# steve-the-bayesian/BOOM

Hardware: AMD Instinct MI355X
Metric: Gibbs sweeps/sec (all chains), n=1e4 p=512 spike-slab (higher is better)
Workload: dtype f64; 1 GPU; BregVsSampler spike-and-slab n=1e4 p=512, 1024 chains per GPU, fp64 (BASELINE configs[1]); chains_per_gpu=1024, true_signals=16, burn_in=1000, parallelism=chains sharded, 1 GPU(s), suf_build=single device MFMA syrk

## Files before the change

boom_amd/csrc/engine.hip:

```cpp
#include "engine_internal.h"

namespace boom_amd {

static thread_local std::string g_error = "";

int fail(int code, const std::string &msg) {
  g_error = msg;
  return code;
}

}

namespace {


const char *status_message(int st) {
  switch (st) {
    case CHAIN_NOT_PD:
      return "The posterior information matrix is not positive definite.  "
             "Check your data or consider adjusting your prior.";
    case CHAIN_NEGATIVE_SS:
      return "Illegal data caused negative sum of squares in "
             "Breg::set_reg_post_params.";
    case CHAIN_ILLEGAL_START:
// ... 1496 lines not shown
  return BA_OK;
}
int read_per_chain(ba_engine *e, const double *dev, int64_t chain, double *out) {
  HIP_TRY(hipStreamSynchronize(e->stream));
  if (chain < 0) HIP_TRY(hipMemcpy(out, dev, (size_t)e->cfg.chains * 8, hipMemcpyDeviceToHost));
  else HIP_TRY(hipMemcpy(out, dev + chain, 8, hipMemcpyDeviceToHost));
  return BA_OK;
}

static int sweep_impl(ba_engine *e, int32_t nsweeps, bool record, int la_half) {
  if (nsweeps < 0) return fail(BA_E_INVALID, "nsweeps must be non-negative");
  int rc = sweep_refusal(e, DATA_REGRESSION);
  if (rc) return rc;
  rc = switch_mode(e, 0, 1.0);
  if (rc) return rc;
  rc = upload_shared(e);
  if (rc) return rc;
  rc = alloc_chain_state(e);
  if (rc) return rc;
  if (record && e->trace_stride > 0 && nsweeps > e->trace_stride)
    return fail(BA_E_INVALID, "nsweeps exceeds the enabled trace length");
  HIP_TRY(e->dmodel.resize(2 * (size_t)e->cfg.chains * ssvs_scalar_layout(64).total));
  SsvsParams P;
  fill_params(e, P);
  if (!record) {
    P.trace_sigsq = P.trace_logp = P.trace_k = nullptr;
    P.rec_idx = nullptr;
    P.rec_beta = nullptr;
    P.trace_stride = 0;
    P.trace_idx = nullptr;
    if (e->trace_stride > 0)
      HIP_TRY(hipMemsetAsync(e->dtrace_idx.ptr, 0, (size_t)e->cfg.chains * 4, e->stream));
  }
  const SsvsLds lay = ssvs_lds_layout(e->p, e->kcap);
  if (lay.total > e->lds_per_cu)
    return fail(BA_E_INVALID, "problem does not fit the LDS working set");
  if (record && e->trace_stride > 0 && la_half < 0)
    HIP_TRY(hipMemsetAsync(e->dtrace_idx.ptr, 0, (size_t)e->cfg.chains * 4, e->stream));
  if (la_half >= 0) {
    const size_t C = (size_t)e->cfg.chains, pp = (size_t)e->p;
    const size_t o1 = (size_t)la_half * C, op = (size_t)la_half * C * pp;
    P.trace_row0 = la_half * e->la_len;
    P.snap_gamma = e->snap_gamma.ptr + op;
    P.snap_beta = e->snap_beta.ptr + op;
    P.snap_sigsq = e->snap_sigsq.ptr + o1;
    P.snap_perm = e->snap_perm.ptr + op;
    P.snap_pos = e->snap_pos.ptr + o1;
    P.snap_fail = e->snap_fail.ptr + o1;
    P.snap_inc = e->snap_inc.ptr + op;
    P.snap_bsum = e->snap_bsum.ptr + op;
    P.snap_bsumsq = e->snap_bsumsq.ptr + op;
    P.snap_acc = e->snap_acc.ptr + (size_t)la_half * C * ACC_COUNT;
  }
#ifndef BA_PIPELINE
#define BA_PIPELINE 1
#endif
  const int resident_per_cu = (int)std::min<size_t>(4, e->lds_per_cu / lay.total);
  const bool pipelined = BA_PIPELINE && nsweeps > 0 && (e->trace_stride == 0 || la_half >= 0) && !e->big_active &&
                         e->cfg.chains <= resident_per_cu * e->cu_count && (!e->kt_enabled || e->kt_overlap);
  if (la_half >= 0 && !pipelined) return fail(BA_E_STATE, "look-ahead batch cannot overlap");
  if (!pipelined) {
    const int C = e->cfg.chains, group = resident_per_cu * e->cu_count;
    const bool groups = BA_PIPELINE && nsweeps > 0 && e->cur_mode != 2 && !e->big_active && C > group &&
                        e->trace_stride == 0 && (!e->kt_enabled || e->kt_overlap);
    if (groups) {
      if (!e->pipe_stream) {
        {
// ... 61 lines not shown
  e->model_ok = true;
  return BA_OK;
}
}

extern "C" {

int ba_sweep(ba_engine *e, int32_t nsweeps) {
  ENGINE_PROLOGUE_NOJOIN(e);
  if (e->la_served < e->la_avail || e->data_kind != DATA_REGRESSION || e->cur_mode != 0) {
    int rcj = pipe_join(e);
    if (rcj) return rcj;
  }
  int rc = la_rewind(e);
  if (rc) return rc;
  return sweep_impl(e, nsweeps, e->la_len <= 1);
}

int ba_set_lookahead(ba_engine *e, int32_t lookahead) {
  ENGINE_PROLOGUE(e);
  if (lookahead < 1) return fail(BA_E_INVALID, "lookahead must be at least 1");
  MUTATE(e);
  if (lookahead > 1) {
    int rc = ba_enable_draws(e, 2 * lookahead);
    if (rc) return rc;
  }
  e->la_len = lookahead;
  e->la_pipe = true;
  return BA_OK;
}

static bool la_can_overlap(const ba_engine *e) {
  if (!BA_PIPELINE || !e->la_pipe || e->big_active || (e->kt_enabled && !e->kt_overlap) || e->kcap <= 0) return false;
  const size_t lds = ssvs_lds_layout(e->p, e->kcap).total;
  if (lds > e->lds_per_cu) return false;
  const int resident_per_cu = (int)std::min<size_t>(4, e->lds_per_cu / lds);
  return e->cfg.chains <= resident_per_cu * e->cu_count;
}

int ba_draw_next(ba_engine *e) {
  ENGINE_PROLOGUE_NOJOIN(e);
  if (e->la_len <= 1) return ba_sweep(e, 1);
  if (e->la_served == e->la_avail) {
    if (e->la_ahead) {
      e->la_slot ^= 1;
      e->la_ahead = false;
      e->la_avail = e->la_served = 0;
      e->la_cache.clear();
      e->la_synced = false;
      e->la_cur_piped = true;
    } else {
      int rc = pipe_join(e);
      if (rc) return rc;
      la_discard(e);
      rc = switch_mode(e, 0, 1.0);
      if (!rc) rc = upload_shared(e);
      if (!rc) rc = alloc_chain_state(e);
      if (rc) return rc;
      if (!e->la_done[0]) {
        HIP_TRY(hipEventCreateWithFlags(&e->la_done[0], hipEventDisableTiming));
        HIP_TRY(hipEventCreateWithFlags(&e->la_done[1], hipEventDisableTiming));
      }
      e->la_slot = 0;
      if (la_can_overlap(e)) {
        rc = la_snap_alloc(e);
        if (!rc) rc = sweep_impl(e, e->la_len, true, 0);
        e->la_cur_piped = true;
// ... 455 lines not shown
```

boom_amd/csrc/ssvs_device.h:

```cpp
#pragma once
#include <hip/hip_runtime.h>

#include "device_rng.h"
#include "diag.h"
#include "ssvs_params.h"

namespace boom_amd {

namespace {

constexpr int WAVE = 64;
#define BA_INF (__builtin_inf())


#define AS_LDS __attribute__((address_space(3)))
typedef AS_LDS double lds_f64;
typedef AS_LDS uint16_t lds_u16;
typedef AS_LDS uint32_t lds_u32;
typedef AS_LDS uint8_t lds_u8;
template <class T>
__device__ __forceinline__ AS_LDS T *to_lds(unsigned char *generic) {
  return (AS_LDS T *)(uintptr_t)generic;
}
#define AS_CONST __attribute__((address_space(4)))
// ... 894 lines not shown
  if (candidate < 0) {
    *status = CHAIN_RNG_BRANCH;
    return;
  }
  double rev;
  {
    const int l2 = P.cm_start[candidate], h2 = P.cm_start[candidate + 1];
    double ans = -BA_INF, tot = 0.0;
    for (int i = l2; i < h2; ++i) {
      const int v = P.cm_idx[i];
      const bool inc = (v == candidate) ? true : ((v == index) ? false : (bool)ch.gam[v]);
      if (!inc) {
        if (v == index) ans = P.cm_cor[i];
        tot += P.cm_cor[i];
      }
    }
    rev = (tot == 0.0) ? 0.0 : ans / tot;
  }
  pe.kind = EV_TRY_LT;
  pe.f1 = index;
  pe.f2 = candidate;
  pe.lfw = log(forward_w);
  pe.lrev = log(rev);
  pe.lu = log(d_runif(rng, 0.0, 1.0));
  pe.check_legal = false;
}

}


enum : int { CMD_EXIT = 0, CMD_EVAL = 1, CMD_UNIF = 2, CMD_DECIDE = 3, CMD_SHUFFLE_DECIDE = 4 };
enum : int { CT_CMD = 0, CT_K = 1, CT_I0 = 2, CT_LOGP = 3, CT_LP = 4, CT_LDV = 5,
             CT_LDA = 6, CT_Q = 7, CT_C = 8, CT_NFLIPS = 9, CT_POS = 10, CT_PERMSEL = 12,
             CT_EVMODE = 13, CT_CUR = 14,
             CT_SLOT0 = 16, CT_SLOT_STRIDE = 6, CT_ROLL = 44, CT_ACC = 48 };
enum : int { SL_F = 0, SL_J = 1, SL_KIND = 2, SL_LOGU = 3, SL_MARGIN = 4, SL_DELTA = 5 };
enum : int { STOP_ACCEPT = 1, STOP_SLOW = 2, STOP_BAD = 3 };

__device__ __forceinline__ void shuffle_targets(const PhiloxKey &key, uint64_t pos,
                                                int p, int tid, int nthreads,
                                                lds_u16 *oth, bool whole_range = false) {
  const int nt = whole_range ? p : p - 1;
  const uint64_t b0 = pos >> 1, b1 = (pos + (uint64_t)(nt - 1)) >> 1;
  for (uint64_t b = b0 + (uint64_t)tid; b <= b1; b += (uint64_t)nthreads) {
    double u[2];
    philox_pair(key, b, &u[0], &u[1]);
#pragma unroll
    for (int h = 0; h < 2; ++h) {
      const long long t = (long long)(2 * b + h) - (long long)pos;
      if (t >= 0 && t < nt) {
        if (whole_range) {
          oth[t] = (uint16_t)(int)floor(0.0 + ((double)p - 0.0) * u[h]);
        } else {
          const int i = p - 1 - (int)t;
          oth[i] = (uint16_t)(int)floor(0.0 + ((double)(i + 1) - 0.0) * u[h]);
        }
      }
    }
  }
}

enum : int { EVM_BATCH = 0, EVM_FILL = 1 };

template <int NB, bool MLVS = false>
__device__ __forceinline__ void eval_share(const SsvsParams &P, Chain &ch,
                                           const Model &M, const PhiloxKey &key,
                                           uint64_t flip_pos, int nflips, int i0,
                                           int evmode, int wave, lds_f64 *ctl,
                                           StampCtx &sx) {
  const int lane = ch.lane;
  SUBSTAMP(sx, 7);
  const int idx = i0 + WAVE * wave + lane;
  if (evmode == EVM_FILL) {
    const bool valid = idx < ch.p;
    const Proposal pr = eval_proposal<NB, true, MLVS>(P, ch, M, valid ? idx : 0, valid, sx, idx - lane);
    if (valid) {
// ... 143 lines not shown
```

boom_amd/csrc/ssvs_kernel.hip:

```cpp
#include "ktimer.h"
#include "ssvs_sweep_body.h"

namespace boom_amd {

__global__ __launch_bounds__(64) void ssvs_logp_kernel(SsvsParams P,
                                                       const uint8_t *gammas,
                                                       int ngamma, double *out,
                                                       int *status_out) {
  extern __shared__ __attribute__((aligned(16))) unsigned char smem[];
  const int which = blockIdx.x, lane = threadIdx.x, p = P.p;
  if (which >= ngamma) return;
  const SsvsLds lay = ssvs_lds_layout(p, P.kcap);
  Chain ch;
  ch.lane = lane;
  ch.p = p;
  bind_lds(ch, smem, lay);
  ch.xty = P.xty;
  ch.DF = P.nobs[0] + P.prior_df;
  ch.ss0q = P.prior_ss + P.yty[0];
  ch.mode = 0;
  ch.sv = ch.sa = ch.sx = 1.0;
  const uint8_t *gg = gammas + (size_t)which * p;
  int k = 0;
  for (int base = 0; base < p; base += WAVE) {
// ... 94 lines not shown
  }
  if (P.snap_gamma) {
    const size_t o = (size_t)chain * (size_t)P.p;
    for (int j = threadIdx.x; j < P.p; j += WAVE * W) {
      P.snap_gamma[o + j] = P.gamma[o + j];
      P.snap_beta[o + j] = P.beta[o + j];
      P.snap_perm[o + j] = P.perm[o + j];
      P.snap_inc[o + j] = P.inc_count[o + j];
      P.snap_bsum[o + j] = P.beta_sum[o + j];
      P.snap_bsumsq[o + j] = P.beta_sumsq[o + j];
    }
    if (threadIdx.x < ACC_COUNT)
      P.snap_acc[(size_t)chain * ACC_COUNT + threadIdx.x] = P.acc[(size_t)chain * ACC_COUNT + threadIdx.x];
    if (threadIdx.x == 0) {
      P.snap_sigsq[chain] = P.sigsq[chain];
      P.snap_pos[chain] = P.rng_pos[chain];
      P.snap_fail[chain] = P.failures[chain];
    }
  }
  ssvs_sweep_body<NB, W, WPE, MLVS>(P, nsweeps, chain, smem);
  if (P.q_out) {
    __syncthreads();
    __threadfence();
    if (threadIdx.x == 0) {
      const int t = atomicAdd(P.q_out + Q_PUSH, 1);
      __hip_atomic_store(P.q_out + Q_READY + t, chain, __ATOMIC_RELEASE, __HIP_MEMORY_SCOPE_AGENT);
    }
  }
}

template <int NB, int W, int WPE, bool MLVS = false>
static hipError_t launch_sweep_t(hipStream_t stream, const SsvsParams &P,
                                 int nsweeps) {
  const SsvsLds lay = ssvs_lds_layout(P.p, NB * 8);
  hipError_t e = hipFuncSetAttribute((const void *)ssvs_sweep_kernel<NB, W, WPE, MLVS>,
                                     hipFuncAttributeMaxDynamicSharedMemorySize,
                                     (int)lay.total);
  if (e != hipSuccess) return e;
  KtScope kt(stream, KT_SSVS);
  hipLaunchKernelGGL((ssvs_sweep_kernel<NB, W, WPE, MLVS>), dim3(P.chain_count), dim3(WAVE * W),
                     lay.total, stream, P, nsweeps);
  return hipGetLastError();
}

hipError_t launch_ssvs_sweep(hipStream_t stream, const SsvsParams &P,
                             int nsweeps) {
  const int key = P.kcap * 10 + P.waves;
#ifndef BA_ONLY_322
  if (P.mode == 3) {
    if (!P.flip_order || !P.wss) return hipErrorInvalidValue;
    switch (P.kcap) {
      case 16: return launch_sweep_t<2, 1, 1, true>(stream, P, nsweeps);
      case 32: return launch_sweep_t<4, 1, 1, true>(stream, P, nsweeps);
      case 48: return launch_sweep_t<6, 1, 1, true>(stream, P, nsweeps);
      case 64: return launch_sweep_t<8, 1, 1, true>(stream, P, nsweeps);
      default: return hipErrorInvalidValue;
    }
  }
#endif
  switch (key) {
#ifdef BA_ONLY_322
    case 322: return launch_sweep_t<4, 2, 2>(stream, P, nsweeps);
    default: return hipErrorInvalidValue;
#else
    case 161: return launch_sweep_t<2, 1, 1>(stream, P, nsweeps);
    case 321: return launch_sweep_t<4, 1, 1>(stream, P, nsweeps);
    case 481: return launch_sweep_t<6, 1, 1>(stream, P, nsweeps);
// ... 63 lines not shown
```

boom_amd/csrc/ssvs_params.h:

```cpp
#pragma once
#include <stdint.h>

namespace boom_amd {

enum ChainStatus : int32_t {
  CHAIN_OK = 0,
  CHAIN_NOT_PD = 1,
  CHAIN_NEGATIVE_SS = 2,
  CHAIN_ILLEGAL_START = 3,
  CHAIN_RNG_BRANCH = 4,
  CHAIN_FORECAST_VARIANCE = 5,
  CHAIN_MODEL_TOO_LARGE = 6,
  CHAIN_NEED_COLUMN = 7,
  CHAIN_NEED_COLUMN_BIG = 8
};
enum { MLVS_ILLEGAL_START = 12 };

enum { SUMMARY_SCALARS = 16 };
enum {
  ACC_SWEEPS = 0,
  ACC_SIGSQ = 1,
  ACC_SIGSQ2 = 2,
  ACC_K = 3,
  ACC_ACCEPTS = 4,
// ... 74 lines not shown
  int32_t trace_stride;
  uint16_t *rec_idx;
  double *rec_beta;
  int32_t rec_cap;

  double *ada_birth, *ada_death;
  uint64_t *ada_iter;
  double ada_step, ada_target;
  int32_t ada_max_flips;
  int32_t *q_in, *q_out;
  int32_t *q_error;
  int32_t trace_row0;
  uint8_t *snap_gamma;
  double *snap_beta, *snap_sigsq, *snap_bsum, *snap_bsumsq, *snap_acc;
  uint16_t *snap_perm;
  uint64_t *snap_pos;
  int32_t *snap_fail;
  uint32_t *snap_inc;
  int32_t adaptive;
  double *ada_ws;

  int32_t big_kcap;
  double *big_model;
  int64_t big_model_stride;
  double *big_xs;
  const double *xty_planes;
  int32_t xty_nplanes;
  int64_t xty_plane_stride;
  const uint16_t *flip_order;
  const double *wss;
};

struct SsvsLds {
  uint32_t Lv, La, rdv, rda, w, bg, ctrl, park, g, perm0, perm1, oth, last, pred, gam, gam0, nbr, total;
};

static inline __host__ __device__ SsvsLds ssvs_lds_layout(int p, int kcap) {
  SsvsLds L;
  const uint32_t nb = (uint32_t)kcap / 8;
  const uint32_t fac = nb * (nb + 1) / 2 * 64 * 8;
  const uint32_t pv = (((uint32_t)p * 2) + 15u) & ~15u;
  uint32_t o = 0;
  L.Lv = o;    o += fac;
  L.La = o;    o += fac;
  L.rdv = o;   o += (uint32_t)kcap * 8;
  L.rda = o;   o += (uint32_t)kcap * 8;
  L.w = o;     o += (uint32_t)kcap * 8;
  L.bg = o;    o += (uint32_t)kcap * 8;
  L.ctrl = o;  o += 512;
  L.park = o;  o += 4 * 512;
  L.g = o;     o += (((uint32_t)kcap * 2) + 15u) & ~15u;
  L.perm0 = o; o += pv;
  L.perm1 = o; o += pv;
  L.oth = o;   o += pv;
  L.last = o;  o += 2 * pv;
  L.pred = o;  o += pv;
  L.gam = o;   o += ((uint32_t)p + 15u) & ~15u;
  L.gam0 = o;  o += ((uint32_t)p + 15u) & ~15u;
  L.nbr = o;   o += ((uint32_t)p + 15u) & ~15u;
  L.total = o;
  return L;
}

struct SsvsBigLds {
  uint32_t tile, rdt, w, y, rd, bst, ctrl, g, gst, perm0, perm1, oth, last, pred, gam, gam0, nbr, total;
};
static inline __host__ __device__ SsvsBigLds ssvs_big_lds_layout(int p, int kcap) {
  SsvsBigLds L;
  const uint32_t pv = (((uint32_t)p * 2) + 15u) & ~15u;
  uint32_t o = 0;
  L.tile = o;  o += 36 * 64 * 8;
  L.rdt = o;   o += 64 * 8;
  L.w = o;     o += (uint32_t)kcap * 8;
  L.y = o;     o += (uint32_t)kcap * 8;
  L.rd = o;    o += (uint32_t)kcap * 8;
  L.bst = o;   o += (uint32_t)kcap * 8;
  L.ctrl = o;  o += 512;
  L.g = o;     o += (((uint32_t)kcap * 2) + 15u) & ~15u;
  L.gst = o;   o += (((uint32_t)kcap * 2) + 15u) & ~15u;
  L.perm0 = o; o += pv;
  L.perm1 = o; o += pv;
  L.oth = o;   o += pv;
  L.last = o;  o += 2 * pv;
  L.pred = o;  o += pv;
  L.gam = o;   o += ((uint32_t)p + 15u) & ~15u;
  L.gam0 = o;  o += ((uint32_t)p + 15u) & ~15u;
  L.nbr = o;   o += ((uint32_t)p + 15u) & ~15u;
  L.total = o;
  return L;
}

struct SsvsAdaLds {
// ... 53 lines not shown
```

boom_amd/csrc/ssvs_sweep_body.h:

```cpp
#pragma once
#include "ssvs_device.h"

namespace boom_amd {

template <int NB, int W, int WPE, bool MLVS = false>
__device__ __forceinline__ void ssvs_sweep_body(SsvsParams P, int nsweeps, const int chain,
                                                unsigned char *smem) {
  constexpr bool SHUFFLE_MASKED = NB >= 6 && W > 1;
  P.V += (size_t)chain * (size_t)P.v_chain_stride;
  if (P.col_valid) {
    P.col_valid += (size_t)chain * (size_t)P.col_words;
    P.v_diag += (size_t)chain * (size_t)P.p;
  }
  int tid_ = threadIdx.x;
  BA_OPAQUE_V(tid_);
  int lane = tid_ & (WAVE - 1);
  const int wave = tid_ >> 6;
  const int p = P.p;
#ifdef BA_PSTAMPS
  long long pst[8];
  pst[0] = (long long)__builtin_readcyclecounter();
#endif
  constexpr int FOLD_Z = 16;
  const bool fold = (W == 1) && P.xty_planes != nullptr;
// ... 1 lines not shown
  double pl[2][FOLD_Z];
  if (fold_early) {
    const double *src = P.xty_planes + (size_t)chain * p;
#pragma unroll
    for (int e = 0; e < 2; ++e) {
      const int j = lane + e * WAVE;
#pragma unroll
      for (int z = 0; z < FOLD_Z; ++z)
        pl[e][z] = (j < p && z < P.xty_nplanes) ? src[(size_t)z * P.xty_plane_stride + j] : 0.0;
    }
  }
  if (P.status[chain] != CHAIN_OK) {
    if (threadIdx.x == 0) {
      P.todo[chain] += nsweeps;
      if (P.ran) P.ran[chain] = 0;
    }
    return;
  }
  int owed_after = 0;
  {
    int total = nsweeps + P.todo[chain];
    if (P.run_limit > 0 && total > P.run_limit) {
      owed_after = total - P.run_limit;
      total = P.run_limit;
    }
    if (total == 0) {
      if (threadIdx.x == 0 && P.ran) P.ran[chain] = 0;
      return;
    }
    nsweeps = total;
  }

  constexpr int KCAP = NB * 8;
  const SsvsLds lay = ssvs_lds_layout(p, KCAP);
  Chain ch;
  ch.lane = lane;
  ch.p = p;
  ch.k = 0;
  bind_lds(ch, smem, lay);
  lds_f64 *ctl = to_lds<double>(smem + lay.ctrl);
  PSTAMP(1);
  ch.xty = P.xty + (size_t)chain * P.xty_stride;
  if (fold_early) {
    double *dst = const_cast<double *>(P.xty) + (size_t)chain * P.xty_stride;
#pragma unroll
    for (int e = 0; e < 2; ++e) {
      const int j = lane + e * WAVE;
      double a = pl[e][0];
#pragma unroll
      for (int z = 1; z < FOLD_Z; ++z)
        if (z < P.xty_nplanes) a += pl[e][z];
      if (j < p) dst[j] = a;
    }
    __builtin_amdgcn_fence(__ATOMIC_RELEASE, "wavefront");
    __builtin_amdgcn_s_waitcnt(0);
  } else if (fold) {
    double *dst = const_cast<double *>(P.xty) + (size_t)chain * P.xty_stride;
    const double *src = P.xty_planes + (size_t)chain * p;
    for (int j = lane; j < p; j += WAVE) {
      double a = src[j];
      for (int z0 = 1; z0 < P.xty_nplanes; z0 += 8) {
        double v[8];
#pragma unroll
        for (int u = 0; u < 8; ++u)
          v[u] = (z0 + u < P.xty_nplanes) ? src[(size_t)(z0 + u) * P.xty_plane_stride + j] : 0.0;
#pragma unroll
        for (int u = 0; u < 8; ++u)
// ... 20 lines not shown
    if (P.slab_scales) { ch.sv = inv; ch.sa = inv; }
  }
  const PhiloxKey key{P.seed_lo, P.seed_hi,
                      (uint32_t)(P.chain_offset + chain), P.stream};

  StampCtx sx_unused;
  sx_unused.last = 0;
  if (W > 1 && wave != 0) {
    sx_unused.last = (long long)__builtin_readcyclecounter();
    for (int i = 0; i < 8; ++i) sx_unused.ph[i] = 0.0;
    for (;;) {
      HSTAMP(sx_unused, 7);
      __syncthreads();
      HSTAMP(sx_unused, 5);
      const int cmd = (int)ctl[CT_CMD];
      if (cmd == CMD_EXIT) break;
      const uint64_t upos = ((AS_LDS const uint64_t *)(ctl + CT_POS))[0];
      if (cmd == CMD_EVAL) {
        Model M;
        M.logp = ctl[CT_LOGP]; M.lp = ctl[CT_LP]; M.ldv = ctl[CT_LDV];
        M.lda = ctl[CT_LDA]; M.Q = ctl[CT_Q]; M.c = ctl[CT_C];
        M.SS = 0; M.pd = true; M.bad = 0;
        ch.k = (int)ctl[CT_K];
        ch.perm = to_lds<uint16_t>(smem + (((int)ctl[CT_PERMSEL]) ? lay.perm1 : lay.perm0));
        bind_slot(ch, P, chain, (int)ctl[CT_CUR]);
        unsigned long long a = (unsigned long long)ch.sc_store;
        asm volatile("" : "+s"(a) : : "memory");
        ch.sc = (c_f64 *)a;
        eval_share<NB, MLVS>(P, ch, M, key, upos, (int)ctl[CT_NFLIPS], (int)ctl[CT_I0],
                             (int)ctl[CT_EVMODE], wave, ctl, sx_unused);
        HSTAMP(sx_unused, 6);
      } else if (cmd == CMD_DECIDE || cmd == CMD_SHUFFLE_DECIDE) {
        if (cmd == CMD_SHUFFLE_DECIDE) {
          shuffle_targets(key, upos, p, threadIdx.x, WAVE * W, ch.oth);
          __syncthreads();
        }
        if (wave == 1) {
          const int sel = (int)ctl[CT_PERMSEL];
          bind_slot(ch, P, chain, (int)ctl[CT_CUR]);
          ch.perm = to_lds<uint16_t>(smem + (sel ? lay.perm1 : lay.perm0));
          ch.perm_alt = to_lds<uint16_t>(smem + (sel ? lay.perm0 : lay.perm1));
          uint64_t fpos = upos;
          if (cmd == CMD_SHUFFLE_DECIDE) {
            parallel_shuffle<SHUFFLE_MASKED>(ch, sx_unused);
            fpos = upos + (uint64_t)(p - 1);
          }
          DecideResult dr;
          decide_walk<MLVS>(ch, key, fpos, (int)ctl[CT_I0], (int)ctl[CT_NFLIPS], dr);
          HSTAMP(sx_unused, 4);
          if (lane == 0) {
            lds_f64 *sl = ctl + CT_SLOT0 + CT_SLOT_STRIDE * 1;
            sl[SL_F] = (double)dr.spos;
            sl[SL_J] = (double)dr.j;
            sl[SL_KIND] = (double)dr.kind;
            sl[SL_LOGU] = dr.logu;
            sl[SL_MARGIN] = dr.margin;
          }
        }
      } else {
        if (p > 1) shuffle_targets(key, upos, p, threadIdx.x, WAVE * W, ch.oth, P.mode == 2);
      }
      HSTAMP(sx_unused, 7);
      __syncthreads();
      HSTAMP(sx_unused, 5);
    }
#if defined(BA_STAMPS) && defined(BA_STAMPS4)
    if (wave == 1 && lane == 0) {
      double *a = P.acc + (size_t)chain * ACC_COUNT;
      for (int i = 0; i < 8; ++i) a[ACC_PHASE0 + i] += sx_unused.ph[i];
    }
#endif
    return;
  }

  uint8_t *g_gamma = P.gamma + (size_t)chain * p;
  uint16_t *g_perm = P.perm + (size_t)chain * p;
  int k = 0;
  int status = CHAIN_OK;
  for (int base = 0; base < p; base += WAVE) {
    const int j = base + lane;
    const int inc = (j < p) ? g_gamma[j] : 0;
    if (j < p) {
      ch.gam[j] = (uint8_t)inc;
      ch.perm[j] = g_perm[j];
      ch.nbr[j] = (uint8_t)((P.cm_start != nullptr) && (P.cm_start[j + 1] > P.cm_start[j]));
    }
    const unsigned long long mask = __ballot(inc != 0);
    const int slot = k + __popcll(mask & ((1ull << lane) - 1ull));
    if (inc && slot < KCAP) ch.g[slot] = (uint16_t)j;
    k += __popcll(mask);
  }
  if (k > KCAP) status = CHAIN_MODEL_TOO_LARGE;
  ch.k = k;
  wave_sync();
  bool aborted = false;
  int need_col = -1;
  int kmax = k;
  int trace_at = (P.trace_row0 >= 0) ? P.trace_row0 : (P.trace_idx ? P.trace_idx[chain] : 0);

  uint64_t pos = uni((uint64_t)P.rng_pos[chain]);
  int failures = uni((int)P.failures[chain]);
  double sigsq = uni((double)P.sigsq[chain]);
  double beta_m = 0.0;
  int gprev = 0, kprev = 0;
  bool beta_valid = false;

  lds_f64 *sum_b = to_lds<double>(smem + lay.park + 512);
  lds_f64 *sum_b2 = to_lds<double>(smem + lay.park + 1024);
  AS_LDS int *sum_n = to_lds<int>(smem + lay.park + 1536);
  AS_LDS int *sum_g = to_lds<int>(smem + lay.park + 1792);
  sum_b[lane] = 0.0; sum_b2[lane] = 0.0; sum_n[lane] = 0; sum_g[lane] = -1;
  if (lane < 8) ctl[CT_ACC + lane] = (lane == ACC_MIN_MARGIN) ? BA_INF : 0.0;
  wave_sync();
#define ACC_ADD(slot, x) do { if (lane == 0) ctl[CT_ACC + (slot)] += (double)(x); } while (0)
#define ACC_MIN(x) do { if (lane == 0) ctl[CT_ACC + ACC_MIN_MARGIN] = fmin(ctl[CT_ACC + ACC_MIN_MARGIN], (x)); } while (0)
  int done = 0;

  const int nflips = P.max_flips;
  STAMP_DECL;
  StampCtx sx;
  sx.last = (long long)__builtin_readcyclecounter();
  for (int i = 0; i < 8; ++i) sx.ph[i] = 0.0;

  Model M;
  M.bad = 0; M.pd = true; M.logp = 0; M.lp = 0; M.ldv = 0; M.lda = 0; M.Q = 0; M.c = 0; M.SS = 0;
  Pending pe;
  pe.kind = EV_INIT; pe.f1 = pe.f2 = -1; pe.lu = 0; pe.lfw = pe.lrev = 0; pe.check_legal = false;
  enum { PH_BEGIN, PH_FLIPS, PH_SWAP, PH_TAIL, PH_JOIN, PH_COMMIT };
  int phase = PH_BEGIN, sweep = 0, i0 = 0;
  bool model_checked = false;
  int perm_sel = 0;
  bool use_table = false;
  int cur = 0, other_var = -1;
  bool other_ok = false, table_valid_other = false;
  const int model_tag_in = P.model_keep ? P.model_tag[chain] : 0;
  const bool model_kept = (model_tag_in & 0xff) == KCAP && status == CHAIN_OK;
  if (model_kept) cur = (model_tag_in >> 8) & 1;
  bind_slot(ch, P, chain, cur);
  bool table_valid = P.table_keep && model_kept && P.table_tag[chain] == model_tag_in;
  int fill_j = 0;
  bool spec = false;
  bool have_dr = false;
  int after_join = PH_COMMIT, spec_status = CHAIN_OK;
  bool commit_pending = false, gam0_fresh = false;
  lds_f64 *park = to_lds<double>(smem + lay.park);
  int stops_prev = table_valid ? 0 : (1 << 20), stops_now = 0;
  uint64_t flip_pos = 0, pos0 = pos;
  WinRng rng;
  rng.init(key, lane, pos);

  PSTAMP(3);
  if (model_kept) {
    {
      const SsvsScalarLayout S = ssvs_scalar_layout(KCAP);
      const double *sc = ch.sc_store + S.scal;
      const double s0 = sc[0], s1 = sc[1], s2 = sc[2], s3 = sc[3], s4 = sc[4], s5 = sc[5], s6 = sc[6], s7 = sc[7];
      restore_model<NB>(ch);
      M.logp = s0; M.lp = s1; M.ldv = s2; M.lda = s3;
      M.Q = s4; M.c = s5; M.SS = s6; M.pd = s7 != 0.0;
      unsigned long long u = (unsigned long long)ch.sc_store;
      asm volatile("s_dcache_inv\n\ts_waitcnt lgkmcnt(0)" : "+s"(u) : : "memory");
      ch.sc = (c_f64 *)u;
    }
    if (P.suf_changed) {
      refactor<true, MLVS>(P, ch, M, sx);
      if (M.bad) status = M.bad;
      else publish_model<NB>(ch, M);
    }
    if (lane == 0) {
      ctl[CT_LOGP] = M.logp; ctl[CT_LP] = M.lp; ctl[CT_LDV] = M.ldv;
      ctl[CT_LDA] = M.lda; ctl[CT_Q] = M.Q; ctl[CT_C] = M.c;
    }
    wave_sync();
    pe.kind = EV_NONE;
  }

  PSTAMP(4);
// ... 109 lines not shown
      if (sweep + (commit_pending ? 1 : 0) >= nsweeps) {
        if (!commit_pending) break;
        phase = PH_COMMIT;
        continue;
      }
      {
        const bool ut = (P.walk_policy != 0) && (stops_prev <= 1 || P.walk_policy == 2);
        const bool mc = model_checked || (M.logp > -BA_INF && M.logp < BA_INF);
        const bool will_fork = nflips > 0 && W > 1 && ut && table_valid && mc && p > 1 && P.walk_policy != 3 && P.mode != 2 && !MLVS;
        if (commit_pending && !will_fork) {
          phase = PH_COMMIT;
          continue;
        }
      }
      STAMP(7);
      TSTAMP(sx, 7);
      if (nflips > 0) {
        if (!gam0_fresh || P.mode) {
          for (int j = lane; j < p; j += WAVE) {
            ch.gam0[j] = ch.gam[j];
            if constexpr (MLVS) ch.perm[j] = P.flip_order[j];
            else if (P.mode) ch.perm[j] = (uint16_t)j;
          }
          gam0_fresh = true;
        }
        TSTAMP(sx, 1);
        pos0 = pos;
        if (!model_checked && M.logp > -BA_INF && M.logp < BA_INF) model_checked = true;
        use_table = (P.walk_policy != 0) && (stops_prev <= 1 || P.walk_policy == 2);
        stops_prev = stops_now;
        stops_now = 0;
        if (W > 1 && use_table && table_valid && model_checked && p > 1 && P.walk_policy != 3 && P.mode != 2 && !MLVS) {
          wave_sync();
          if (lane == 0) {
            ctl[CT_CMD] = (double)CMD_SHUFFLE_DECIDE;
            ctl[CT_I0] = 0.0;
            ctl[CT_NFLIPS] = (double)nflips;
            ctl[CT_PERMSEL] = (double)perm_sel;
            ctl[CT_CUR] = (double)cur;
            ((AS_LDS uint64_t *)(ctl + CT_POS))[0] = pos;
          }
          __syncthreads();
          shuffle_targets(key, pos, p, threadIdx.x, WAVE * W, ch.oth);
          __syncthreads();
          {
            lds_u16 *tmp = ch.perm;
            ch.perm = ch.perm_alt;
            ch.perm_alt = tmp;
            perm_sel ^= 1;
          }
          flip_pos = pos + (uint64_t)(p - 1);
          pos = flip_pos + (uint64_t)nflips;
          TSTAMP(sx, 2);
          spec = true;
          spec_status = CHAIN_OK;
          park[lane] = beta_m;
          if (lane == 0) {
            ctl[CT_ROLL + 0] = sigsq;
            ctl[CT_ROLL + 1] = (double)failures;
            ctl[CT_ROLL + 2] = beta_valid ? 1.0 : 0.0;
          }
          i0 = 0;
          phase = commit_pending ? PH_COMMIT : PH_SWAP;
          STAMP(1);
          continue;
        }
        if constexpr (MLVS) {
          wave_sync();
          flip_pos = pos;
          pos = flip_pos + (uint64_t)nflips;
          if (!(M.logp > -BA_INF && M.logp < BA_INF)) { status = MLVS_ILLEGAL_START; aborted = true; }
        } else {
        if (W > 1) {
          if (lane == 0) {
            ctl[CT_CMD] = (double)CMD_UNIF;
            ((AS_LDS uint64_t *)(ctl + CT_POS))[0] = pos;
          }
// ... 27 lines not shown
                if (!inc && column_missing(P, j)) { status = CHAIN_NEED_COLUMN; need_col = j; aborted = true; break; }
                apply_flip(ch, j);
              }
            }
            pe.kind = EV_INIT;
            pe.check_legal = true;
          }
        }
        }
      }
      i0 = 0;
      phase = PH_FLIPS;
      continue;
    }

    if (phase == PH_FLIPS) {
      if (nflips == 0 || i0 >= nflips) {
        phase = PH_SWAP;
        continue;
      }
      if (use_table && table_valid) {
        DecideResult dr;
        if (W > 1) {
          if (!have_dr) {
          if (lane == 0) {
            ctl[CT_CMD] = (double)CMD_DECIDE;
            ctl[CT_I0] = (double)i0;
            ctl[CT_NFLIPS] = (double)nflips;
            ctl[CT_PERMSEL] = (double)perm_sel;
            ctl[CT_CUR] = (double)cur;
            ((AS_LDS uint64_t *)(ctl + CT_POS))[0] = flip_pos;
          }
          __syncthreads();
          __syncthreads();
          }
          have_dr = false;
          const lds_f64 *sl = ctl + CT_SLOT0 + CT_SLOT_STRIDE * 1;
          dr.spos = uni((int)sl[SL_F]);
          dr.j = uni((int)sl[SL_J]);
          dr.kind = uni((int)sl[SL_KIND]);
          dr.logu = uni((double)sl[SL_LOGU]);
          dr.margin = uni((double)sl[SL_MARGIN]);
        } else {
          decide_walk<MLVS>(ch, key, flip_pos, i0, nflips, dr);
        }
        ACC_MIN(dr.margin);
        STAMP(3);
        if (dr.spos < 0) {
          ACC_ADD(ACC_PROPOSALS, nflips - i0);
          i0 = nflips;
          continue;
        }
        ACC_ADD(ACC_PROPOSALS, dr.spos + 1 - i0);
        ++stops_now;
        i0 = dr.spos + 1;
        if (dr.kind == STOP_BAD) {
          status = CHAIN_NEGATIVE_SS;
          break;
        }
        if (!ch.gam[dr.j] && ch.k >= KCAP) {
          status = CHAIN_MODEL_TOO_LARGE;
          aborted = true;
          break;
        }
        if (!ch.gam[dr.j] && column_missing(P, dr.j)) {
          status = CHAIN_NEED_COLUMN;
// ... 86 lines not shown
      if (kind == STOP_ACCEPT) {
        pe.kind = EV_FORCE;
      } else {
        pe.kind = EV_TRY_GE;
        pe.lu = uni((double)sl[SL_LOGU]);
      }
      i0 += nprop;
      continue;
    }

    if (phase == PH_SWAP) {
      TSTAMP(sx, 7);
      rng.set_pos(pos);
      if (nflips > 0) propose_swap(P, ch, rng, pe, &status);
      pos = rng.get_pos();
      phase = PH_TAIL;
      if (spec && (pe.kind != EV_NONE || status != CHAIN_OK)) {
        spec_status = status;
        status = CHAIN_OK;
        after_join = PH_TAIL;
        phase = PH_JOIN;
      }
      STAMP(4);
      TSTAMP(sx, 3);
      continue;
    }

    if (phase == PH_JOIN) {
      __syncthreads();
      spec = false;
      const lds_f64 *sl = ctl + CT_SLOT0 + CT_SLOT_STRIDE * 1;
      if ((int)sl[SL_F] < 0) {
        ACC_MIN(sl[SL_MARGIN]);
        ACC_ADD(ACC_PROPOSALS, nflips);
        status = spec_status;
        phase = after_join;
        if (after_join == PH_COMMIT && status == CHAIN_OK) {
          commit_pending = true;
          phase = PH_BEGIN;
        }
      } else {
        pos = flip_pos + (uint64_t)nflips;
        beta_m = park[lane];
        sigsq = ctl[CT_ROLL + 0];
        failures = (int)ctl[CT_ROLL + 1];
        beta_valid = ctl[CT_ROLL + 2] != 0.0;
        pe.kind = EV_NONE; pe.f1 = pe.f2 = -1; pe.lfw = pe.lrev = 0.0; pe.check_legal = false;
        have_dr = true;
        phase = PH_FLIPS;
      }
      STAMP(3);
      continue;
    }

    if (phase == PH_COMMIT) {
      TSTAMP(sx, 7);
      k = ch.k;
      gprev = (lane < k) ? (int)ch.g[lane] : 0;
      kprev = k;
      kmax = k > kmax ? k : kmax;
      {
        const int gnow = (lane < k) ? gprev : -1;
        const int gold = sum_g[lane];
        if (__any(gnow != gold)) {
          const int n_old = sum_n[lane];
          if (gold >= 0 && n_old) {
            const size_t o = (size_t)chain * p + gold;
// ... 58 lines not shown
        continue;
      }
      failures = 0;
      const double z = draw_normals(rng, k);
      pos = uni(rng.get_pos());
      TSTAMP(sx, 5);
      const double sigma = P.mode ? 1.0 : sqrt(sigsq);
      double y = (lane < k) ? ch.w[lane] + sigma * z : 0.0;
      const double rdm = (lane < k) ? ch.rdv[lane] : 0.0;
#pragma nounroll
      for (int ib = (k - 1) >> 3; ib >= 0; --ib) {
        double lr[8];
        const int base = bidx(ib * 8, lane < ib * 8 + 8 ? lane : 0);
#pragma unroll
        for (int t = 0; t < 8; ++t) lr[t] = ch.Lv[base + t * 8];
#pragma unroll
        for (int t = 7; t >= 0; --t) {
          const int i = ib * 8 + t;
          if (i < k) {
            const double xi = bcast_u(y * rdm, i);
            if (lane == i) y = xi;
            else if (lane < i) y -= lr[t] * xi;
          }
        }
      }
      beta_m = y;
      beta_valid = true;
      TSTAMP(sx, 6);
    } else if (P.draw_beta) {
      beta_valid = true;
    }
    STAMP(6);
    after_join = PH_COMMIT;
    phase = spec ? PH_JOIN : PH_COMMIT;
  }

  PSTAMP(5);
  if (W > 1) {
    if (lane == 0) ctl[CT_CMD] = (double)CMD_EXIT;
    __syncthreads();
  }

  wave_sync();
#ifndef BA_STAMPS
  double *acc_row = P.acc + (size_t)chain * ACC_COUNT;
  const double acc_old = (lane < 8) ? acc_row[lane] : 0.0;
#endif
  if (sum_g[lane] >= 0 && sum_n[lane]) {
    const size_t o = (size_t)chain * p + sum_g[lane];
    P.inc_count[o] += (unsigned)sum_n[lane];
    P.beta_sum[o] += sum_b[lane];
    P.beta_sumsq[o] += sum_b2[lane];
  }
  wave_sync();
  {
    const lds_u8 *gsrc = aborted ? ch.gam0 : ch.gam;
    const lds_u16 *psrc = (aborted && p > 1) ? ch.perm_alt : ch.perm;
    for (int j = lane; j < p; j += WAVE) {
      g_gamma[j] = gsrc[j];
      g_perm[j] = psrc[j];
    }
    if (aborted) pos = pos0;
  }
  if (beta_valid) {
    double *g_beta = P.beta + (size_t)chain * p;
    for (int j = lane; j < p; j += WAVE) g_beta[j] = 0.0;
// ... 55 lines not shown
```

Baseline: 57.06 million sweeps/s.

## Double-buffer shuffle targets and prefetch next sweep's shuffle during speculation

Adds a second LDS buffer for the shuffle-target array. When the chain is speculating, wave 0 uses its idle time at the end of a sweep to precompute the next sweep's Philox shuffle targets into the spare buffer, so the following CMD_SHUFFLE_DECIDE can skip regenerating them. It also lets a mid-walk CMD_DECIDE re-fork speculation (REFORK) instead of waiting for the helper wave, and corrects the proposal count on join to nflips - i0. The cost is extra LDS use, capped at a quarter of a CU, plus added control-flow complexity and the risk that a stale prefetch is consumed.

```diff
diff --git a/boom_amd/csrc/engine.hip b/boom_amd/csrc/engine.hip
--- a/boom_amd/csrc/engine.hip
+++ b/boom_amd/csrc/engine.hip
@@ -1552,7 +1552,7 @@
     if (e->trace_stride > 0)
       HIP_TRY(hipMemsetAsync(e->dtrace_idx.ptr, 0, (size_t)e->cfg.chains * 4, e->stream));
   }
-  const SsvsLds lay = ssvs_lds_layout(e->p, e->kcap);
+  const SsvsLds lay = ssvs_lds_layout(e->p, e->kcap, e->waves);
   if (lay.total > e->lds_per_cu)
     return fail(BA_E_INVALID, "problem does not fit the LDS working set");
   if (record && e->trace_stride > 0 && la_half < 0)
@@ -1680,7 +1680,7 @@
 
 static bool la_can_overlap(const ba_engine *e) {
   if (!BA_PIPELINE || !e->la_pipe || e->big_active || (e->kt_enabled && !e->kt_overlap) || e->kcap <= 0) return false;
-  const size_t lds = ssvs_lds_layout(e->p, e->kcap).total;
+  const size_t lds = ssvs_lds_layout(e->p, e->kcap, e->waves).total;
   if (lds > e->lds_per_cu) return false;
   const int resident_per_cu = (int)std::min<size_t>(4, e->lds_per_cu / lds);
   return e->cfg.chains <= resident_per_cu * e->cu_count;
diff --git a/boom_amd/csrc/ssvs_device.h b/boom_amd/csrc/ssvs_device.h
--- a/boom_amd/csrc/ssvs_device.h
+++ b/boom_amd/csrc/ssvs_device.h
@@ -950,16 +950,19 @@
 enum : int { CMD_EXIT = 0, CMD_EVAL = 1, CMD_UNIF = 2, CMD_DECIDE = 3, CMD_SHUFFLE_DECIDE = 4 };
 enum : int { CT_CMD = 0, CT_K = 1, CT_I0 = 2, CT_LOGP = 3, CT_LP = 4, CT_LDV = 5,
              CT_LDA = 6, CT_Q = 7, CT_C = 8, CT_NFLIPS = 9, CT_POS = 10, CT_PERMSEL = 12,
-             CT_EVMODE = 13, CT_CUR = 14,
+             CT_EVMODE = 13, CT_CUR = 14, CT_OTH = 15,
              CT_SLOT0 = 16, CT_SLOT_STRIDE = 6, CT_ROLL = 44, CT_ACC = 48 };
 enum : int { SL_F = 0, SL_J = 1, SL_KIND = 2, SL_LOGU = 3, SL_MARGIN = 4, SL_DELTA = 5 };
 enum : int { STOP_ACCEPT = 1, STOP_SLOW = 2, STOP_BAD = 3 };
 
 __device__ __forceinline__ void shuffle_targets(const PhiloxKey &key, uint64_t pos,
                                                 int p, int tid, int nthreads,
-                                                lds_u16 *oth, bool whole_range = false) {
+                                                lds_u16 *oth, bool whole_range = false,
+                                                uint32_t blk_first = 0, uint32_t blk_count = 1u << 30) {
   const int nt = whole_range ? p : p - 1;
-  const uint64_t b0 = pos >> 1, b1 = (pos + (uint64_t)(nt - 1)) >> 1;
+  const uint64_t b0 = (pos >> 1) + (uint64_t)blk_first;
+  uint64_t b1 = (pos + (uint64_t)(nt - 1)) >> 1;
+  if (blk_count < (1u << 30) && b0 + (uint64_t)blk_count <= b1) b1 = b0 + (uint64_t)blk_count - 1;
   for (uint64_t b = b0 + (uint64_t)tid; b <= b1; b += (uint64_t)nthreads) {
     double u[2];
     philox_pair(key, b, &u[0], &u[1]);
diff --git a/boom_amd/csrc/ssvs_kernel.hip b/boom_amd/csrc/ssvs_kernel.hip
--- a/boom_amd/csrc/ssvs_kernel.hip
+++ b/boom_amd/csrc/ssvs_kernel.hip
@@ -150,7 +150,7 @@
 template <int NB, int W, int WPE, bool MLVS = false>
 static hipError_t launch_sweep_t(hipStream_t stream, const SsvsParams &P,
                                  int nsweeps) {
-  const SsvsLds lay = ssvs_lds_layout(P.p, NB * 8);
+  const SsvsLds lay = ssvs_lds_layout(P.p, NB * 8, W);
   hipError_t e = hipFuncSetAttribute((const void *)ssvs_sweep_kernel<NB, W, WPE, MLVS>,
                                      hipFuncAttributeMaxDynamicSharedMemorySize,
                                      (int)lay.total);
diff --git a/boom_amd/csrc/ssvs_params.h b/boom_amd/csrc/ssvs_params.h
--- a/boom_amd/csrc/ssvs_params.h
+++ b/boom_amd/csrc/ssvs_params.h
@@ -130,10 +130,12 @@
 };
 
 struct SsvsLds {
-  uint32_t Lv, La, rdv, rda, w, bg, ctrl, park, g, perm0, perm1, oth, last, pred, gam, gam0, nbr, total;
-};
-
-static inline __host__ __device__ SsvsLds ssvs_lds_layout(int p, int kcap) {
+  uint32_t Lv, La, rdv, rda, w, bg, ctrl, park, g, perm0, perm1, oth, last, pred, gam, gam0, nbr, oth1, total;
+};
+
+enum : uint32_t { SSVS_LDS_QUARTER_CU = 40u * 1024u };
+
+static inline __host__ __device__ SsvsLds ssvs_lds_layout(int p, int kcap, int waves = 1) {
   SsvsLds L;
   const uint32_t nb = (uint32_t)kcap / 8;
   const uint32_t fac = nb * (nb + 1) / 2 * 64 * 8;
@@ -156,6 +158,8 @@
   L.gam = o;   o += ((uint32_t)p + 15u) & ~15u;
   L.gam0 = o;  o += ((uint32_t)p + 15u) & ~15u;
   L.nbr = o;   o += ((uint32_t)p + 15u) & ~15u;
+  L.oth1 = L.oth;
+  if (waves > 1 && o + pv <= SSVS_LDS_QUARTER_CU) { L.oth1 = o; o += pv; }
   L.total = o;
   return L;
 }
diff --git a/boom_amd/csrc/ssvs_sweep_body.h b/boom_amd/csrc/ssvs_sweep_body.h
--- a/boom_amd/csrc/ssvs_sweep_body.h
+++ b/boom_amd/csrc/ssvs_sweep_body.h
@@ -57,7 +57,13 @@
   }
 
   constexpr int KCAP = NB * 8;
-  const SsvsLds lay = ssvs_lds_layout(p, KCAP);
+  const SsvsLds lay = ssvs_lds_layout(p, KCAP, W);
+#ifndef BA_PRE_BLOCKS
+#define BA_PRE_BLOCKS (1u << 30)
+#endif
+  constexpr uint32_t PRE_BLOCKS = BA_PRE_BLOCKS;
+  constexpr bool PRE_ALL = PRE_BLOCKS >= (1u << 30);
+  const bool prefetch = W > 1 && !MLVS && lay.oth1 != lay.oth;
   Chain ch;
   ch.lane = lane;
   ch.p = p;
@@ -144,8 +150,15 @@
         HSTAMP(sx_unused, 6);
       } else if (cmd == CMD_DECIDE || cmd == CMD_SHUFFLE_DECIDE) {
         if (cmd == CMD_SHUFFLE_DECIDE) {
-          shuffle_targets(key, upos, p, threadIdx.x, WAVE * W, ch.oth);
-          __syncthreads();
+          const int ow = (int)ctl[CT_OTH];
+          ch.oth = to_lds<uint16_t>(smem + ((ow & 1) ? lay.oth1 : lay.oth));
+          if (!(ow & 2)) {
+            shuffle_targets(key, upos, p, threadIdx.x, WAVE * W, ch.oth);
+            __syncthreads();
+          } else if (!PRE_ALL) {
+            shuffle_targets(key, upos, p, threadIdx.x, WAVE * W, ch.oth, false, PRE_BLOCKS);
+            __syncthreads();
+          }
         }
         if (wave == 1) {
           const int sel = (int)ctl[CT_PERMSEL];
@@ -170,6 +183,7 @@
           }
         }
       } else {
+        ch.oth = to_lds<uint16_t>(smem + ((((int)ctl[CT_OTH]) & 1) ? lay.oth1 : lay.oth));
         if (p > 1) shuffle_targets(key, upos, p, threadIdx.x, WAVE * W, ch.oth, P.mode == 2);
       }
       HSTAMP(sx_unused, 7);
@@ -223,6 +237,7 @@
   AS_LDS int *sum_g = to_lds<int>(smem + lay.park + 1792);
   sum_b[lane] = 0.0; sum_b2[lane] = 0.0; sum_n[lane] = 0; sum_g[lane] = -1;
   if (lane < 8) ctl[CT_ACC + lane] = (lane == ACC_MIN_MARGIN) ? BA_INF : 0.0;
+  if (lane == 0) ctl[CT_OTH] = 0.0;
   wave_sync();
 #define ACC_ADD(slot, x) do { if (lane == 0) ctl[CT_ACC + (slot)] += (double)(x); } while (0)
 #define ACC_MIN(x) do { if (lane == 0) ctl[CT_ACC + ACC_MIN_MARGIN] = fmin(ctl[CT_ACC + ACC_MIN_MARGIN], (x)); } while (0)
@@ -252,9 +267,16 @@
   bool table_valid = P.table_keep && model_kept && P.table_tag[chain] == model_tag_in;
   int fill_j = 0;
   bool spec = false;
+#ifndef BA_REFORK
+#define BA_REFORK 1
+#endif
+  constexpr bool REFORK = BA_REFORK != 0;
   bool have_dr = false;
   int after_join = PH_COMMIT, spec_status = CHAIN_OK;
   bool commit_pending = false, gam0_fresh = false;
+  int oth_sel = 0;
+  bool pre_ok = false;
+  uint64_t pre_tag = 0;
   lds_f64 *park = to_lds<double>(smem + lay.park);
   int stops_prev = table_valid ? 0 : (1 << 20), stops_now = 0;
   uint64_t flip_pos = 0, pos0 = pos;
@@ -430,17 +452,29 @@
         stops_now = 0;
         if (W > 1 && use_table && table_valid && model_checked && p > 1 && P.walk_policy != 3 && P.mode != 2 && !MLVS) {
           wave_sync();
+          const bool ready = prefetch && pre_ok && pre_tag == pos;
+          pre_ok = false;
+          if (ready) {
+            oth_sel ^= 1;
+            ch.oth = to_lds<uint16_t>(smem + (oth_sel ? lay.oth1 : lay.oth));
+          }
           if (lane == 0) {
             ctl[CT_CMD] = (double)CMD_SHUFFLE_DECIDE;
             ctl[CT_I0] = 0.0;
             ctl[CT_NFLIPS] = (double)nflips;
             ctl[CT_PERMSEL] = (double)perm_sel;
             ctl[CT_CUR] = (double)cur;
+            ctl[CT_OTH] = (double)(oth_sel | (ready ? 2 : 0));
             ((AS_LDS uint64_t *)(ctl + CT_POS))[0] = pos;
           }
           __syncthreads();
-          shuffle_targets(key, pos, p, threadIdx.x, WAVE * W, ch.oth);
-          __syncthreads();
+          if (!ready) {
+            shuffle_targets(key, pos, p, threadIdx.x, WAVE * W, ch.oth);
+            __syncthreads();
+          } else if (!PRE_ALL) {
+            shuffle_targets(key, pos, p, threadIdx.x, WAVE * W, ch.oth, false, PRE_BLOCKS);
+            __syncthreads();
+          }
           {
             lds_u16 *tmp = ch.perm;
             ch.perm = ch.perm_alt;
@@ -534,6 +568,19 @@
             ((AS_LDS uint64_t *)(ctl + CT_POS))[0] = flip_pos;
           }
           __syncthreads();
+          if (REFORK && model_checked && p > 1 && P.walk_policy != 3 && P.mode != 2 && !MLVS) {
+            spec = true;
+            spec_status = CHAIN_OK;
+            park[lane] = beta_m;
+            if (lane == 0) {
+              ctl[CT_ROLL + 0] = sigsq;
+              ctl[CT_ROLL + 1] = (double)failures;
+              ctl[CT_ROLL + 2] = beta_valid ? 1.0 : 0.0;
+            }
+            phase = PH_SWAP;
+            STAMP(1);
+            continue;
+          }
           __syncthreads();
           }
           have_dr = false;
@@ -686,7 +733,7 @@
       const lds_f64 *sl = ctl + CT_SLOT0 + CT_SLOT_STRIDE * 1;
       if ((int)sl[SL_F] < 0) {
         ACC_MIN(sl[SL_MARGIN]);
-        ACC_ADD(ACC_PROPOSALS, nflips);
+        ACC_ADD(ACC_PROPOSALS, nflips - i0);
         status = spec_status;
         phase = after_join;
         if (after_join == PH_COMMIT && status == CHAIN_OK) {
@@ -811,6 +858,14 @@
     }
     STAMP(6);
     after_join = PH_COMMIT;
+    if (prefetch && spec && nflips > 0 && sweep + 1 < nsweeps) {
+      TSTAMP(sx, 7);
+      shuffle_targets(key, pos, p, lane, WAVE, to_lds<uint16_t>(smem + (oth_sel ? lay.oth : lay.oth1)),
+                      false, 0, PRE_BLOCKS);
+      pre_tag = pos;
+      pre_ok = true;
+      TSTAMP(sx, 1);
+    }
     phase = spec ? PH_JOIN : PH_COMMIT;
   }
 
```

Result: slower. 56.46 million sweeps/s (-1.1%).
